# Lumina-Group/libzkp

Measured on NVIDIA B200. Metric: groth16_bn254_proofs_per_sec_batched, higher is better.
Workload: dtype u256 (8x32-bit Montgomery limbs, integer)

## Files before the change

libzkp_b200/csrc/ec.cuh:

```cuda
#pragma once
#include "field.cuh"

namespace lzkp {

template <class F>
struct Affine {
    F x, y;
    LZ_HD bool is_inf() const { return x.is_zero() && y.is_zero(); }
    LZ_HD static Affine inf() { return Affine{F::zero(), F::zero()}; }
    LZ_HD Affine neg() const { return Affine{x, y.neg()}; }
};

template <class F>
struct XYZZ {
    F x, y, zz, zzz;
    LZ_HD bool is_inf() const { return zz.is_zero(); }
    LZ_HD static XYZZ inf() { return XYZZ{F::one(), F::one(), F::zero(), F::zero()}; }
    LZ_HD static XYZZ from_affine(const Affine<F> &p) {
        if (p.is_inf()) return inf();
        return XYZZ{p.x, p.y, F::one(), F::one()};
    }
    LZ_HD XYZZ neg() const { return XYZZ{x, y.neg(), zz, zzz}; }

    LZ_COLD static XYZZ dbl_affine(const Affine<F> &p) {
        if (p.y.is_zero()) return inf();
        F U = p.y.dbl(), V = U.sqr(), W = U * V, S = p.x * V;
        F xx = p.x.sqr(), M = xx.dbl() + xx;
        XYZZ r;
        r.x = M.sqr() - S.dbl();
        r.y = F::msub(M, S - r.x, W, p.y);
        r.zz = V;
        r.zzz = W;
        return r;
    }
    LZ_HD void dbl() {
        if (is_inf()) return;
        if (y.is_zero()) { *this = inf(); return; }
        F U = y.dbl(), V = U.sqr(), W = U * V, S = x * V;
        F xx = x.sqr(), M = xx.dbl() + xx;
        F X3 = M.sqr() - S.dbl();
        F Y3 = F::msub(M, S - X3, W, y);
        x = X3; y = Y3;
        zz = V * zz;
        zzz = W * zzz;
    }
    LZ_COLD void dbl_cold() { dbl(); }
    LZ_COLD void add_cold(const XYZZ &q) { add(q); }
    LZ_COLD void madd_cold(const Affine<F> &p) { madd(p); }
    LZ_HD void madd(const Affine<F> &p) {
        if (p.is_inf()) return;
        if (is_inf()) { *this = from_affine(p); return; }
        F U2 = p.x * zz, S2 = p.y * zzz;
        F Pp = U2 - x, R = S2 - y;
        if (Pp.is_zero()) {
            if (R.is_zero()) *this = dbl_affine(p);
            else *this = inf();
            return;
        }
        F PP = Pp.sqr(), PPP = Pp * PP, Q = x * PP;
        F X3 = R.sqr() - PPP - Q.dbl();
        F Y3 = F::msub(R, Q - X3, y, PPP);
        x = X3; y = Y3;
        zz = zz * PP;
        zzz = zzz * PPP;
    }
    LZ_HD void madd_lazy(const Affine<F> &p) {
        if (p.is_inf()) return;
        if (zz.is_zero_2p()) { *this = from_affine(p); return; }
        F U2 = F::mul_lazy(p.x, zz), S2 = F::mul_lazy(p.y, zzz);
        F Pp = F::sub_2p(U2, x), R = F::sub_2p(S2, y);
        if (Pp.is_zero_2p()) {
            if (R.is_zero_2p()) *this = dbl_affine(p);
            else *this = inf();
            return;
        }
        F PP = Pp.sqr_lazy();
        F PPP = F::mul_lazy(Pp, PP), Q = F::mul_lazy(x, PP);
        F RR = R.sqr_lazy();
        F X3 = F::sub_2p(F::sub_2p(RR, PPP), F::add_2p(Q, Q));
        F Y3 = F::msub_lazy(R, F::sub_2p(Q, X3), y, PPP);
        x = X3; y = Y3;
        zz = F::mul_lazy(zz, PP);
        zzz = F::mul_lazy(zzz, PPP);
    }
    LZ_HD XYZZ canonical() const { return XYZZ{x.canonical(), y.canonical(), zz.canonical(), zzz.canonical()}; }
    LZ_HD void add(const XYZZ &q) {
        if (q.is_inf()) return;
        if (is_inf()) { *this = q; return; }
        F U1 = x * q.zz, U2 = q.x * zz, S1 = y * q.zzz, S2 = q.y * zzz;
        F Pp = U2 - U1, R = S2 - S1;
        if (Pp.is_zero()) {
            if (R.is_zero()) dbl_cold();
            else *this = inf();
            return;
        }
        F PP = Pp.sqr(), PPP = Pp * PP, Q = U1 * PP;
        F X3 = R.sqr() - PPP - Q.dbl();
        F Y3 = F::msub(R, Q - X3, S1, PPP);
        x = X3; y = Y3;
        zz = zz * q.zz * PP;
        zzz = zzz * q.zzz * PPP;
    }
    LZ_COLD Affine<F> to_affine() const {
        if (is_inf()) return Affine<F>::inf();
        F t = (zz * zzz).inverse();
        return Affine<F>{x * (t * zzz), y * (t * zz)};
    }
};

template <class F, int LIMBS>
LZ_COLD XYZZ<F> scalar_mul_window(const XYZZ<F> &p, const uint32_t (&k)[LIMBS]) {
    constexpr int NW = LIMBS * 8;
    static_assert(NW <= 64, "carry mask is 64 bits");
    XYZZ<F> T[8];
    T[0] = p;
    T[1] = p;
    T[1].dbl_cold();
#pragma unroll 1
    for (int i = 2; i < 8; i++) {
        T[i] = T[i - 1];
        T[i].add_cold(p);
    }
    uint64_t carries = 0;
    uint32_t c = 0;
#pragma unroll 1
    for (int i = 0; i < NW; i++) {
        const uint32_t v = ((k[i >> 3] >> ((i & 7) * 4)) & 15u) + c;
        c = v >= 8u ? 1u : 0u;
        carries |= (uint64_t)c << i;
    }
    XYZZ<F> acc = XYZZ<F>::inf();
#pragma unroll 1
    for (int i = NW; i >= 0; i--) {
        acc.dbl_cold(); acc.dbl_cold(); acc.dbl_cold(); acc.dbl_cold();
        int d;
        if (i == NW) d = (int)c;
        else {
            const uint32_t cin = i ? (uint32_t)(carries >> (i - 1)) & 1u : 0u, cout = (uint32_t)(carries >> i) & 1u;
            d = (int)(((k[i >> 3] >> ((i & 7) * 4)) & 15u) + cin) - (int)(16u * cout);
        }
        if (d != 0) {
            XYZZ<F> q = T[(d < 0 ? -d : d) - 1];
            if (d < 0) q.y = q.y.neg();
            acc.add_cold(q);
        }
    }
    return acc;
}
template <class F>
LZ_COLD XYZZ<F> scalar_mul(const XYZZ<F> &p, const Fr &k_canonical) {
    return scalar_mul_window<F, 8>(p, k_canonical.l);
}

struct GlvSplit {
    uint32_t k1[4], k2[4];
    bool neg1, neg2, ok;
};
template <int NO, int NA, int NB>
LZ_HD void mul_limbs(uint32_t (&out)[NO], const uint32_t (&a)[NA], const uint32_t (&b)[NB]) {
    uint64_t acc = 0, hi = 0;
#pragma unroll
    for (int k = 0; k < NO; k++) {
#pragma unroll
        for (int i = 0; i < NA; i++) {
            int j = k - i;
            if (j < 0 || j >= NB) continue;
            uint64_t p = (uint64_t)a[i] * b[j];
            acc += (uint32_t)p;
            hi += p >> 32;
        }
        out[k] = (uint32_t)acc;
        acc = (acc >> 32) + hi;
        hi = 0;
    }
}
LZ_HD GlvSplit glv_split(const Fr &k) {
    const uint32_t G1C[5] = {0x00ff6565u, 0x5398fd03u, 0xa773d2d2u, 0x4ccef014u, 0x00000002u};
    const uint32_t G2C[3] = {0xc7e0b3d7u, 0xd91d232eu, 0x00000002u};
    const uint32_t A1[4] = {0x7d4f1128u, 0x8211bbebu, 0xeeb859fcu, 0x6f4d8248u};
    const uint32_t A2[2] = {0x94d213e3u, 0x89d32568u};
    const uint32_t B2[4] = {0x1221250bu, 0x0be4e154u, 0xeeb859fdu, 0x6f4d8248u};
    uint32_t t13[13], t11[11], c1[5], c2[3];
    mul_limbs<13, 8, 5>(t13, k.l, G1C);
#pragma unroll
    for (int i = 0; i < 5; i++) c1[i] = t13[8 + i];
    mul_limbs<11, 8, 3>(t11, k.l, G2C);
#pragma unroll
    for (int i = 0; i < 3; i++) c2[i] = t11[8 + i];
    uint32_t p1[8], p2[8], p3[8], p4[8], k1[8], k2[8], t[8];
    mul_limbs<8, 5, 4>(p1, c1, A1);
    mul_limbs<8, 3, 2>(p2, c2, A2);
    mul_limbs<8, 5, 2>(p3, c1, A2);
    mul_limbs<8, 3, 4>(p4, c2, B2);
    sub8(t, k.l, p1);
    sub8(k1, t, p2);
    sub8(k2, p3, p4);
    GlvSplit o;
    o.neg1 = (k1[7] >> 31) != 0;
    o.neg2 = (k2[7] >> 31) != 0;
    uint32_t zero[8] = {0, 0, 0, 0, 0, 0, 0, 0};
    if (o.neg1) { sub8(t, zero, k1);
#pragma unroll
        for (int i = 0; i < 8; i++) k1[i] = t[i]; }
    if (o.neg2) { sub8(t, zero, k2);
#pragma unroll
        for (int i = 0; i < 8; i++) k2[i] = t[i]; }
    o.ok = (k1[4] | k1[5] | k1[6] | k1[7] | k2[4] | k2[5] | k2[6] | k2[7]) == 0;
#pragma unroll
    for (int i = 0; i < 4; i++) { o.k1[i] = k1[i]; o.k2[i] = k2[i]; }
    return o;
}
template <class F>
LZ_COLD XYZZ<F> scalar_mul_u128(const XYZZ<F> &p, const uint32_t (&k)[4]) {
    return scalar_mul_window<F, 4>(p, k);
}

static LZ_COLD XYZZ<Fq> scalar_mul_glv64(const XYZZ<Fq> &p, const uint32_t (&k)[4]) {
    XYZZ<Fq> T[8];
    T[0] = p;
    T[1] = p;
    T[1].dbl_cold();
#pragma unroll 1
    for (int i = 2; i < 8; i++) {
        T[i] = T[i - 1];
        T[i].add_cold(p);
    }
    Fq beta;
#pragma unroll
    for (int i = 0; i < 8; i++) beta.l[i] = FqParams::BETA(i);
    uint32_t carries[2] = {0, 0}, top[2] = {0, 0};
#pragma unroll 1
    for (int h = 0; h < 2; h++) {
        uint32_t c = 0;
#pragma unroll 1
        for (int i = 0; i < 16; i++) {
            const uint32_t v = ((k[2 * h + (i >> 3)] >> ((i & 7) * 4)) & 15u) + c;
            c = v >= 8u ? 1u : 0u;
            carries[h] |= c << i;
        }
        top[h] = c;
    }
    XYZZ<Fq> acc = XYZZ<Fq>::inf();
#pragma unroll 1
    for (int i = 16; i >= 0; i--) {
        acc.dbl_cold(); acc.dbl_cold(); acc.dbl_cold(); acc.dbl_cold();
#pragma unroll 1
        for (int h = 0; h < 2; h++) {
            int d;
            if (i == 16) d = (int)top[h];
            else {
                const uint32_t cin = i ? (carries[h] >> (i - 1)) & 1u : 0u, cout = (carries[h] >> i) & 1u;
                d = (int)(((k[2 * h + (i >> 3)] >> ((i & 7) * 4)) & 15u) + cin) - (int)(16u * cout);
            }
            if (d != 0) {
                XYZZ<Fq> q = T[(d < 0 ? -d : d) - 1];
                if (h) q.x = q.x * beta;
                if (d < 0) q.y = q.y.neg();
                acc.add_cold(q);
            }
        }
    }
    return acc;
}
LZ_HD Fr glv_lambda_mont() {
    const uint32_t v[8] = {0x55fcd653u, 0x0363f299u, 0x5fc1e200u, 0x73e7950bu, 0x576d9d24u, 0xc5fce83eu, 0xa1c3a4d4u, 0x059c805du};
    Fr r;
#pragma unroll
    for (int i = 0; i < 8; i++) r.l[i] = v[i];
    return r;
}
LZ_HD Fr glv64_coefficient(const uint32_t (&k)[4]) {
    Fr k1 = Fr::zero(), k2 = Fr::zero();
    k1.l[0] = k[0]; k1.l[1] = k[1];
    k2.l[0] = k[2]; k2.l[1] = k[3];
    return k1 + k2 * glv_lambda_mont();
}

using G1Affine = Affine<Fq>;
using G2Affine = Affine<Fq2>;
using G1XYZZ = XYZZ<Fq>;
using G2XYZZ = XYZZ<Fq2>;

static LZ_COLD bool g1_on_curve(const G1Affine &p) {
    if (p.is_inf()) return true;
    Fq b3;
#pragma unroll
    for (int i = 0; i < 8; i++) b3.l[i] = FqParams::B3(i);
    return p.y.sqr() == p.x.sqr() * p.x + b3;
}
static LZ_COLD bool g2_on_curve(const G2Affine &p) {
    if (p.is_inf()) return true;
    Fq2 b;
#pragma unroll
    for (int i = 0; i < 8; i++) { b.c0.l[i] = FqParams::G2B_C0(i); b.c1.l[i] = FqParams::G2B_C1(i); }
    return p.y.sqr() == p.x.sqr() * p.x + b;
}

}
```

libzkp_b200/csrc/field.cuh:

```cuda
#pragma once
#include <stdint.h>

#if defined(__CUDACC__)
#define LZ_HD __host__ __device__ __forceinline__
#define LZ_COLD __host__ __device__ __noinline__
#else
#define LZ_HD inline
#define LZ_COLD inline
#endif
#define LZ_CONST_ARRAY(NAME, ...)                                   \
    LZ_HD static constexpr uint32_t NAME(int i) {                   \
        const uint32_t v[8] = {__VA_ARGS__};                        \
        return v[i];                                                \
    }

#include "bn254_constants.cuh"

namespace lzkp {


LZ_HD void row_mul(uint32_t (&D)[8], uint32_t s0, uint32_t s1, uint32_t s2, uint32_t s3, uint32_t k) {
    const uint32_t s[4] = {s0, s1, s2, s3};
#pragma unroll
    for (int t = 0; t < 4; t++) {
// ... 340 lines not shown
        "addc.cc.u32 %7, %7, %17;\n\t"
        "addc.u32 %8, %18, %20;"
        : "+r"(mid[0]), "+r"(mid[1]), "+r"(mid[2]), "+r"(mid[3]), "+r"(mid[4]), "+r"(mid[5]), "+r"(mid[6]), "+r"(mid[7]),
          "=r"(mid[8]), "=&r"(junk)
        : "r"(x[0]), "r"(x[1]), "r"(x[2]), "r"(x[3]), "r"(x[4]), "r"(x[5]), "r"(x[6]), "r"(x[7]), "r"(c), "r"(n & 1u), "r"(n));
    asm("add.cc.u32 %0, %12, %24;\n\t"
        "addc.cc.u32 %1, %13, %25;\n\t"
        "addc.cc.u32 %2, %14, %26;\n\t"
        "addc.cc.u32 %3, %15, %27;\n\t"
        "addc.cc.u32 %4, %16, %28;\n\t"
        "addc.cc.u32 %5, %17, %29;\n\t"
        "addc.cc.u32 %6, %18, %30;\n\t"
        "addc.cc.u32 %7, %19, %31;\n\t"
        "addc.cc.u32 %8, %20, %32;\n\t"
        "addc.cc.u32 %9, %21, 0;\n\t"
        "addc.cc.u32 %10, %22, 0;\n\t"
        "addc.u32 %11, %23, 0;"
        : "=r"(T[4]), "=r"(T[5]), "=r"(T[6]), "=r"(T[7]), "=r"(T[8]), "=r"(T[9]), "=r"(T[10]), "=r"(T[11]), "=r"(T[12]),
          "=r"(T[13]), "=r"(T[14]), "=r"(T[15])
        : "r"(L[4]), "r"(L[5]), "r"(L[6]), "r"(L[7]), "r"(H[0]), "r"(H[1]), "r"(H[2]), "r"(H[3]), "r"(H[4]), "r"(H[5]),
          "r"(H[6]), "r"(H[7]),
          "r"(mid[0]), "r"(mid[1]), "r"(mid[2]), "r"(mid[3]), "r"(mid[4]), "r"(mid[5]), "r"(mid[6]), "r"(mid[7]), "r"(mid[8]));
#pragma unroll
    for (int i = 0; i < 4; i++) T[i] = L[i];
#else
    {
        uint64_t cy = n & 1u;
        for (int i = 0; i < 8; i++) {
            cy += (uint64_t)mid[i] + (M[i] ^ n);
            mid[i] = (uint32_t)cy;
            cy >>= 32;
        }
        mid[8] = (uint32_t)(c + n + cy);
        for (int i = 0; i < 4; i++) T[i] = L[i];
        cy = 0;
        for (int i = 4; i < 16; i++) {
            const uint32_t base = i < 8 ? L[i] : H[i - 8];
            cy += (uint64_t)base + (i - 4 < 9 ? mid[i - 4] : 0u);
            T[i] = (uint32_t)cy;
            cy >>= 32;
        }
    }
#endif
}

LZ_HD uint32_t red_shift_row(uint32_t &A0, uint32_t (&D)[8], uint32_t p1, uint32_t p3, uint32_t p5, uint32_t p7,
                             uint32_t inv) {
    uint32_t m;
#ifdef __CUDA_ARCH__
    asm("add.cc.u32 %0, %0, %2;\n\t"
        "mul.lo.u32 %9, %0, %14;\n\t"
        "madc.lo.cc.u32 %1, %10, %9, %3;\n\t"
        "madc.hi.cc.u32 %2, %10, %9, %4;\n\t"
        "madc.lo.cc.u32 %3, %11, %9, %5;\n\t"
        "madc.hi.cc.u32 %4, %11, %9, %6;\n\t"
        "madc.lo.cc.u32 %5, %12, %9, %7;\n\t"
        "madc.hi.cc.u32 %6, %12, %9, %8;\n\t"
        "madc.lo.cc.u32 %7, %13, %9, 0;\n\t"
        "madc.hi.u32 %8, %13, %9, 0;"
        : "+r"(A0), "+r"(D[0]), "+r"(D[1]), "+r"(D[2]), "+r"(D[3]), "+r"(D[4]), "+r"(D[5]), "+r"(D[6]), "+r"(D[7]), "=&r"(m)
        : "r"(p1), "r"(p3), "r"(p5), "r"(p7), "r"(inv));
#else
    const uint32_t s[4] = {p1, p3, p5, p7};
    uint64_t c = (uint64_t)A0 + D[1];
    A0 = (uint32_t)c;
    c >>= 32;
    m = A0 * inv;
    for (int t = 0; t < 4; t++) {
        uint64_t pr = (uint64_t)s[t] * m;
        uint32_t alo = t < 3 ? D[2 * t + 2] : 0, ahi = t < 3 ? D[2 * t + 3] : 0;
        uint64_t lo = (uint64_t)alo + (uint32_t)pr + c;
        uint64_t hi = (uint64_t)ahi + (uint32_t)(pr >> 32) + (lo >> 32);
        D[2 * t] = (uint32_t)lo;
        D[2 * t + 1] = (uint32_t)hi;
        c = hi >> 32;
    }
#endif
    return m;
}

template <class P>
LZ_HD void wide_fix_negative(uint32_t (&T)[16], uint32_t neg) {
    uint32_t hi[8], pm[8], fix[8];
#pragma unroll
    for (int i = 0; i < 8; i++) { hi[i] = T[8 + i]; pm[i] = neg ? P::MOD(i) : 0u; }
    add8(fix, hi, pm);
#pragma unroll
    for (int i = 0; i < 8; i++) T[8 + i] = fix[i];
}

template <class P>
struct alignas(16) Fp {
    uint32_t l[8];

    LZ_HD static Fp zero() {
        Fp r;
#pragma unroll
        for (int i = 0; i < 8; i++) r.l[i] = 0;
        return r;
    }
    LZ_HD static Fp one() {
        Fp r;
#pragma unroll
        for (int i = 0; i < 8; i++) r.l[i] = P::ONE(i);
        return r;
    }
    LZ_HD static Fp modulus() {
        Fp r;
#pragma unroll
        for (int i = 0; i < 8; i++) r.l[i] = P::MOD(i);
        return r;
    }
    LZ_HD static Fp r2() {
        Fp r;
#pragma unroll
        for (int i = 0; i < 8; i++) r.l[i] = P::R2(i);
        return r;
    }
    LZ_HD bool is_zero() const {
        uint32_t o = 0;
#pragma unroll
        for (int i = 0; i < 8; i++) o |= l[i];
        return o == 0;
    }
    LZ_HD bool operator==(const Fp &b) const {
        uint32_t o = 0;
#pragma unroll
        for (int i = 0; i < 8; i++) o |= l[i] ^ b.l[i];
        return o == 0;
    }
    LZ_HD bool operator!=(const Fp &b) const { return !(*this == b); }

    LZ_HD static Fp reduce_once(const uint32_t (&x)[8]) {
        Fp m = modulus(), d, r;
        uint32_t bw = sub8(d.l, x, m.l);
#pragma unroll
        for (int i = 0; i < 8; i++) r.l[i] = bw ? x[i] : d.l[i];
        return r;
    }
    LZ_HD friend Fp operator+(const Fp &a, const Fp &b) {
        uint32_t s[8];
        add8(s, a.l, b.l);
        return reduce_once(s);
    }
    LZ_HD friend Fp operator-(const Fp &a, const Fp &b) {
        Fp d, e, m = modulus(), r;
        uint32_t bw = sub8(d.l, a.l, b.l);
        add8(e.l, d.l, m.l);
#pragma unroll
        for (int i = 0; i < 8; i++) r.l[i] = bw ? e.l[i] : d.l[i];
        return r;
    }
    LZ_HD Fp neg() const {
        Fp m = modulus(), d, r;
        sub8(d.l, m.l, l);
        bool z = is_zero();
#pragma unroll
        for (int i = 0; i < 8; i++) r.l[i] = z ? 0u : d.l[i];
        return r;
    }
    LZ_HD Fp dbl() const { return *this + *this; }

    LZ_HD friend Fp operator*(const Fp &a, const Fp &b) { return reduce_once(mul_lazy(a, b).l); }
    LZ_HD Fp sqr() const { return reduce_once(sqr_lazy().l); }
    LZ_HD static Fp reduce_wide(const uint32_t (&T)[16]) { return reduce_once(reduce_wide_lazy(T).l); }
    LZ_HD static Fp msub(const Fp &a, const Fp &b, const Fp &c, const Fp &d) { return reduce_once(msub_lazy(a, b, c, d).l); }

    LZ_HD static Fp mul_lazy(const Fp &a, const Fp &b) {
        uint32_t X[8], Y[8];
        uint32_t m, c;
        row_mul(X, a.l[0], a.l[2], a.l[4], a.l[6], b.l[0]);
        row_mul(Y, a.l[1], a.l[3], a.l[5], a.l[7], b.l[0]);
        m = X[0] * P::INV;
        row_mad(Y, P::MOD(1), P::MOD(3), P::MOD(5), P::MOD(7), m);
        c = row_mad(X, P::MOD(0), P::MOD(2), P::MOD(4), P::MOD(6), m);
        Y[7] += c;
#pragma unroll
        for (int i = 1; i < 8; i++) {
            if (i & 1) {
                row_mad_shift(Y[0], X, a.l[1], a.l[3], a.l[5], a.l[7], b.l[i]);
                c = row_mad(Y, a.l[0], a.l[2], a.l[4], a.l[6], b.l[i]);
                X[7] += c;
                m = Y[0] * P::INV;
                row_mad(X, P::MOD(1), P::MOD(3), P::MOD(5), P::MOD(7), m);
                c = row_mad(Y, P::MOD(0), P::MOD(2), P::MOD(4), P::MOD(6), m);
                X[7] += c;
            } else {
                row_mad_shift(X[0], Y, a.l[1], a.l[3], a.l[5], a.l[7], b.l[i]);
                c = row_mad(X, a.l[0], a.l[2], a.l[4], a.l[6], b.l[i]);
                Y[7] += c;
                m = X[0] * P::INV;
                row_mad(Y, P::MOD(1), P::MOD(3), P::MOD(5), P::MOD(7), m);
                c = row_mad(X, P::MOD(0), P::MOD(2), P::MOD(4), P::MOD(6), m);
                Y[7] += c;
            }
        }
        uint32_t hi[8];
#pragma unroll
        for (int j = 0; j < 7; j++) hi[j] = Y[j + 1];
        hi[7] = 0;
        Fp s;
        add8(s.l, X, hi);
        return s;
    }
    LZ_HD Fp sqr_lazy() const {
#ifdef LZKP_SQR_AS_MUL
        return mul_lazy(*this, *this);
#endif
        uint32_t d[8], e[8];
        d[0] = l[0] << 1;
        e[0] = 0;
#pragma unroll
        for (int i = 1; i < 8; i++) { d[i] = (l[i] << 1) | (l[i - 1] >> 31); e[i] = l[i] << 1; }
        uint32_t t0 = 0, t1 = 0, t2 = 0, m[8];
        Fp r;
#pragma unroll
        for (int k = 0; k < 15; k++) {
#pragma unroll
            for (int i = 0; i < 8; i++) {
                const int j = k - i;
                if (j < i || j > 7) continue;
                if (j == i) mac3(t0, t1, t2, l[i], l[i]);
                else if (j == i + 1) mac3(t0, t1, t2, l[i], e[j]);
                else mac3(t0, t1, t2, l[i], d[j]);
            }
            if (k < 8) {
#pragma unroll
                for (int i = 0; i < k; i++) mac3(t0, t1, t2, m[i], P::MOD(k - i));
                m[k] = t0 * P::INV;
                mac3(t0, t1, t2, m[k], P::MOD(0));
            } else {
#pragma unroll
                for (int i = k - 7; i < 8; i++) mac3(t0, t1, t2, m[i], P::MOD(k - i));
                r.l[k - 8] = t0;
            }
            t0 = t1; t1 = t2; t2 = 0;
        }
        r.l[7] = t0;
        return r;
    }
    LZ_HD static Fp reduce_wide_lazy(const uint32_t (&T)[16]) {
        uint32_t X[8], Y[8];
        uint32_t m, c;
#pragma unroll
        for (int j = 0; j < 8; j++) X[j] = T[j];
        m = X[0] * P::INV;
        row_mul(Y, P::MOD(1), P::MOD(3), P::MOD(5), P::MOD(7), m);
        c = row_mad(X, P::MOD(0), P::MOD(2), P::MOD(4), P::MOD(6), m);
        Y[7] += c;
#pragma unroll
        for (int i = 1; i < 8; i++) {
            if (i & 1) {
                m = red_shift_row(Y[0], X, P::MOD(1), P::MOD(3), P::MOD(5), P::MOD(7), P::INV);
                c = row_mad(Y, P::MOD(0), P::MOD(2), P::MOD(4), P::MOD(6), m);
                X[7] += c;
            } else {
                m = red_shift_row(X[0], Y, P::MOD(1), P::MOD(3), P::MOD(5), P::MOD(7), P::INV);
                c = row_mad(X, P::MOD(0), P::MOD(2), P::MOD(4), P::MOD(6), m);
                Y[7] += c;
            }
        }
        uint32_t hi[8], th[8], u[8];
#pragma unroll
        for (int j = 0; j < 7; j++) hi[j] = Y[j + 1];
        hi[7] = 0;
#pragma unroll
        for (int j = 0; j < 8; j++) th[j] = T[8 + j];
        add8(u, X, hi);
        Fp s_;
        add8(s_.l, u, th);
        return s_;
    }
    LZ_HD static Fp msub_lazy(const Fp &a, const Fp &b, const Fp &c, const Fp &d) {
        uint32_t t0[16], t1[16];
        mul_wide(t0, a.l, b.l);
        mul_wide(t1, c.l, d.l);
        const uint32_t bw = sub16(t0, t0, t1);
        wide_fix_negative<P>(t0, bw);
        return reduce_wide_lazy(t0);
    }
    LZ_HD static Fp sub_2p(const Fp &a, const Fp &b) {
        Fp d, e, r;
        uint32_t bw = sub8(d.l, a.l, b.l);
        add8(e.l, d.l, modulus2().l);
#pragma unroll
        for (int i = 0; i < 8; i++) r.l[i] = bw ? e.l[i] : d.l[i];
        return r;
    }
    LZ_HD static Fp add_2p(const Fp &a, const Fp &b) {
        uint32_t s[8];
        Fp d, r;
        add8(s, a.l, b.l);
        uint32_t bw = sub8(d.l, s, modulus2().l);
#pragma unroll
        for (int i = 0; i < 8; i++) r.l[i] = bw ? s[i] : d.l[i];
        return r;
    }
    LZ_HD bool is_zero_2p() const {
        uint32_t z = 0, q = 0;
#pragma unroll
        for (int i = 0; i < 8; i++) { z |= l[i]; q |= l[i] ^ P::MOD(i); }
        return z == 0 || q == 0;
    }
    LZ_HD Fp canonical() const { return reduce_once(l); }
    LZ_HD static Fp modulus2() {
        Fp r;
#pragma unroll
        for (int i = 0; i < 8; i++) r.l[i] = (P::MOD(i) << 1) | (i ? P::MOD(i - 1) >> 31 : 0u);
        return r;
    }

    LZ_HD static Fp from_canonical(const Fp &c) { return c * r2(); }
    LZ_HD Fp to_canonical() const {
        Fp o = zero();
        o.l[0] = 1;
        return *this * o;
    }
    LZ_COLD Fp inverse() const {
        if (is_zero()) return zero();
        uint32_t u[8], v[8], x1[8], x2[8];
        const Fp m = modulus();
#pragma unroll
        for (int i = 0; i < 8; i++) { u[i] = l[i]; v[i] = m.l[i]; x1[i] = 0; x2[i] = 0; }
        x1[0] = 1;
        auto is_one = [](const uint32_t (&a)[8]) {
            uint32_t o = a[0] ^ 1u;
#pragma unroll
            for (int i = 1; i < 8; i++) o |= a[i];
            return o == 0;
        };
        auto shr1 = [](uint32_t (&a)[8]) {
#pragma unroll
            for (int i = 0; i < 7; i++) a[i] = (a[i] >> 1) | (a[i + 1] << 31);
            a[7] >>= 1;
        };
        auto halve_mod = [&](uint32_t (&x)[8]) {
            if (x[0] & 1u) { uint32_t t[8]; add8(t, x, m.l); 
#pragma unroll
                for (int i = 0; i < 8; i++) x[i] = t[i]; }
            shr1(x);
        };
        auto sub_mod = [&](uint32_t (&x)[8], const uint32_t (&y)[8]) {
            uint32_t d[8], e[8];
            uint32_t bw = sub8(d, x, y);
            add8(e, d, m.l);
#pragma unroll
            for (int i = 0; i < 8; i++) x[i] = bw ? e[i] : d[i];
        };
#pragma unroll 1
        while (!is_one(u) && !is_one(v)) {
#pragma unroll 1
            while (!(u[0] & 1u)) { shr1(u); halve_mod(x1); }
#pragma unroll 1
            while (!(v[0] & 1u)) { shr1(v); halve_mod(x2); }
            uint32_t d[8];
            if (sub8(d, u, v) == 0) {
#pragma unroll
                for (int i = 0; i < 8; i++) u[i] = d[i];
                sub_mod(x1, x2);
            } else {
                sub8(d, v, u);
#pragma unroll
                for (int i = 0; i < 8; i++) v[i] = d[i];
                sub_mod(x2, x1);
            }
        }
        Fp r, r3;
        const bool uu = is_one(u);
#pragma unroll
        for (int i = 0; i < 8; i++) { r.l[i] = uu ? x1[i] : x2[i]; r3.l[i] = P::R3(i); }
        return r * r3;
    }
    LZ_HD static bool gt_canonical(const Fp &a, const Fp &b) {
        uint32_t d[8];
        return sub8(d, b.l, a.l) != 0;
    }
};

using Fr = Fp<FrParams>;
using Fq = Fp<FqParams>;

struct Fq2;
#if !defined(LZKP_FQ2_INLINE) && defined(__CUDA_ARCH__)
static __device__ __noinline__ Fq2 fq2_mul_call(Fq2 a, Fq2 b);
static __device__ __noinline__ Fq2 fq2_sqr_call(Fq2 a);
#endif
struct Fq2 {
    Fq c0, c1;
    LZ_HD static Fq2 zero() { return Fq2{Fq::zero(), Fq::zero()}; }
    LZ_HD static Fq2 one() { return Fq2{Fq::one(), Fq::zero()}; }
    LZ_HD bool is_zero() const { return c0.is_zero() && c1.is_zero(); }
    LZ_HD bool operator==(const Fq2 &b) const { return c0 == b.c0 && c1 == b.c1; }
    LZ_HD bool operator!=(const Fq2 &b) const { return !(*this == b); }
    LZ_HD friend Fq2 operator+(const Fq2 &a, const Fq2 &b) { return Fq2{a.c0 + b.c0, a.c1 + b.c1}; }
    LZ_HD friend Fq2 operator-(const Fq2 &a, const Fq2 &b) { return Fq2{a.c0 - b.c0, a.c1 - b.c1}; }
    LZ_HD Fq2 neg() const { return Fq2{c0.neg(), c1.neg()}; }
    LZ_HD Fq2 dbl() const { return Fq2{c0.dbl(), c1.dbl()}; }
    LZ_HD friend Fq2 operator*(const Fq2 &a, const Fq2 &b) {
#if !defined(LZKP_FQ2_INLINE) && defined(__CUDA_ARCH__)
        return fq2_mul_call(a, b);
#elif defined(LZKP_FQ2_SCHOOLBOOK)
        return Fq2{a.c0 * b.c0 - a.c1 * b.c1, a.c0 * b.c1 + a.c1 * b.c0};
#else
        Fq v0 = a.c0 * b.c0, v1 = a.c1 * b.c1;
        Fq s = (a.c0 + a.c1) * (b.c0 + b.c1);
        return Fq2{v0 - v1, s - v0 - v1};
#endif
    }
    LZ_HD Fq2 sqr() const {
#if !defined(LZKP_FQ2_INLINE) && defined(__CUDA_ARCH__)
        return fq2_sqr_call(*this);
#endif
        Fq m = c0 * c1;
        return Fq2{(c0 + c1) * (c0 - c1), m.dbl()};
    }
    LZ_HD static Fq2 msub(const Fq2 &a, const Fq2 &b, const Fq2 &c, const Fq2 &d) { return a * b - c * d; }
    LZ_HD Fq2 inverse() const {
        Fq n = (c0.sqr() + c1.sqr()).inverse();
        return Fq2{c0 * n, (c1 * n).neg()};
    }
};
LZ_HD Fq2 fq2_mul_lazy(const Fq2 &a, const Fq2 &b) {
    uint32_t t0[16], t1[16], t2[16], sa[8], sb[8];
    mul_wide(t0, a.c0.l, b.c0.l);
    mul_wide(t1, a.c1.l, b.c1.l);
    add8(sa, a.c0.l, a.c1.l);
    add8(sb, b.c0.l, b.c1.l);
    mul_wide(t2, sa, sb);
    sub16(t2, t2, t0);
    sub16(t2, t2, t1);
    const uint32_t bw = sub16(t0, t0, t1);
    uint32_t hi[8], pm[8], fix[8];
#pragma unroll
    for (int i = 0; i < 8; i++) { hi[i] = t0[8 + i]; pm[i] = bw ? FqParams::MOD(i) : 0u; }
    add8(fix, hi, pm);
#pragma unroll
    for (int i = 0; i < 8; i++) t0[8 + i] = fix[i];
    return Fq2{Fq::reduce_wide(t0), Fq::reduce_wide(t2)};
}
#if !defined(LZKP_FQ2_INLINE) && defined(__CUDA_ARCH__)
static __device__ __noinline__ Fq2 fq2_mul_call(Fq2 a, Fq2 b) { return fq2_mul_lazy(a, b); }
static __device__ __noinline__ Fq2 fq2_sqr_call(Fq2 a) {
    Fq m = a.c0 * a.c1;
    return Fq2{(a.c0 + a.c1) * (a.c0 - a.c1), m.dbl()};
}
#endif

}
```

libzkp_b200/csrc/msm_batch.cu:

```cuda
#include <algorithm>
#include <cstdlib>
#include "tables.h"
#include "dev_util.cuh"

#ifndef LZKP_G2_MINB
#define LZKP_G2_MINB 6
#endif
#ifndef LZKP_G1_MINB
#define LZKP_G1_MINB 4
#endif
#define LZKP_G2_MINB_SEL(F) (sizeof(F) == sizeof(::lzkp::Fq) ? LZKP_G1_MINB : LZKP_G2_MINB)
namespace lzkp {

template <class F, int BLOCK, class DigT>
__global__ void __launch_bounds__(BLOCK, LZKP_G2_MINB_SEL(F)) k_msm_batch(const Affine<F> *__restrict__ table, uint32_t N,
                                                     const uint32_t *__restrict__ unit_dig,
                                                     const uint32_t *__restrict__ unit_tbl,
                                                     const uint2 *__restrict__ items, const DigT *__restrict__ dig,
                                                     uint32_t P, XYZZ<F> *__restrict__ partial) {
    const uint32_t p = blockIdx.x * BLOCK + threadIdx.x, item = blockIdx.y;
    if (p >= P) return;
    const uint2 range = items[item];
    constexpr bool lazy = sizeof(F) == sizeof(Fq);
    XYZZ<F> acc = XYZZ<F>::inf();
    int d = dig[(size_t)__ldg(unit_dig + range.x) * P + p];
    Affine<F> pt = Affine<F>::inf();
    if (d) pt = gather_point(table, N, __ldg(unit_tbl + range.x), d);
    for (uint32_t u = range.x; u < range.y; u++) {
        int dn = 0;
        Affine<F> ptn = Affine<F>::inf();
        if (u + 1 < range.y) {
            dn = dig[(size_t)__ldg(unit_dig + u + 1) * P + p];
            if (dn) ptn = gather_point(table, N, __ldg(unit_tbl + u + 1), dn);
        }
        if (d) {
            if constexpr (lazy) acc.madd_lazy(pt);
            else acc.madd(pt);
        }
        d = dn;
        pt = ptn;
    }
    if constexpr (lazy) acc = acc.canonical();
    st_vec(partial + (size_t)item * P + p, acc);
}
template <class F>
__global__ void __launch_bounds__(128) k_msm_reduce1(XYZZ<F> *partial, const uint2 *msm_items, uint32_t P, uint32_t G) {
    uint32_t p = blockIdx.x * blockDim.x + threadIdx.x, q = blockIdx.y, g = blockIdx.z;
    if (p >= P) return;
    uint2 r = msm_items[q];
    if (r.x + g >= r.y) return;
    XYZZ<F> acc = ld_vec(partial + (size_t)(r.x + g) * P + p);
    for (uint32_t it = r.x + g + G; it < r.y; it += G) acc.add_cold(ld_vec(partial + (size_t)it * P + p));
    st_vec(partial + (size_t)(r.x + g) * P + p, acc);
}
template <class F>
__global__ void __launch_bounds__(128) k_msm_reduce(const XYZZ<F> *partial, const uint2 *msm_items, uint32_t P,
                                                    uint32_t G, XYZZ<F> *out) {
    uint32_t p = blockIdx.x * blockDim.x + threadIdx.x, q = blockIdx.y;
    if (p >= P) return;
    uint2 r = msm_items[q];
    uint32_t end = min(r.y, r.x + G);
    XYZZ<F> acc = XYZZ<F>::inf();
    for (uint32_t it = r.x; it < end; it++) acc.add_cold(ld_vec(partial + (size_t)it * P + p));
    st_vec(out + (size_t)q * P + p, acc);
}

template <class F>
__global__ void __launch_bounds__(128) k_msm_fold(XYZZ<F> *partial, const uint2 *msm_items, uint32_t P, uint32_t half,
                                                  XYZZ<F> *out) {
    uint32_t p = blockIdx.x * blockDim.x + threadIdx.x, q = blockIdx.y, g = blockIdx.z;
    if (p >= P) return;
    const uint2 r = msm_items[q];
    const uint32_t live = min(r.y - r.x, 2 * half);
    if (g >= live) {
        if (half == 1 && g == 0) st_vec(out + (size_t)q * P + p, XYZZ<F>::inf());
        return;
    }
    XYZZ<F> acc = ld_vec(partial + (size_t)(r.x + g) * P + p);
    if (g + half < live) acc.add_cold(ld_vec(partial + (size_t)(r.x + g + half) * P + p));
    if (half == 1) st_vec(out + (size_t)q * P + p, acc);
    else st_vec(partial + (size_t)(r.x + g) * P + p, acc);
}

template <class F, int T>
__global__ void __launch_bounds__(T) k_msm_reduce_tree(const XYZZ<F> *__restrict__ partial, const uint2 *__restrict__ msm_items,
                                                       uint32_t P, XYZZ<F> *__restrict__ out) {
    __shared__ uint4 raw[T * sizeof(XYZZ<F>) / 16];
    XYZZ<F> *sm = reinterpret_cast<XYZZ<F> *>(raw);
    const uint32_t p = blockIdx.x, q = blockIdx.y, t = threadIdx.x;
    const uint2 r = msm_items[q];
    XYZZ<F> acc = XYZZ<F>::inf();
    for (uint32_t it = r.x + t; it < r.y; it += T) acc.add_cold(ld_vec(partial + (size_t)it * P + p));
    st_vec(sm + t, acc);
    __syncthreads();
    for (uint32_t s = T / 2; s > 0; s >>= 1) {
        if (t < s) {
            XYZZ<F> a = ld_vec(sm + t);
            a.add_cold(ld_vec(sm + t + s));
            st_vec(sm + t, a);
        }
        __syncthreads();
    }
    if (t == 0) st_vec(out + (size_t)q * P + p, ld_vec(sm));
}

}

namespace lzkp {
namespace eng {
uint32_t small_batch_limit() {
    static const uint32_t v = [] {
        const char *e = getenv("LZKP_SMALL_BATCH");
        return e ? (uint32_t)atoi(e) : 512u;
    }();
    return v;
}

int batch_msm_g1_resident(uint32_t dig_bytes, uint32_t *out) {
    int dev = 0, sms = 0, per_sm = 0;
    CUDA_TRY(cudaGetDevice(&dev));
    CUDA_TRY(cudaDeviceGetAttribute(&sms, cudaDevAttrMultiProcessorCount, dev));
    if (dig_bytes == 2) CUDA_TRY(cudaOccupancyMaxActiveBlocksPerMultiprocessor(&per_sm, k_msm_batch<Fq, 128, int16_t>, 128, 0));
    else CUDA_TRY(cudaOccupancyMaxActiveBlocksPerMultiprocessor(&per_sm, k_msm_batch<Fq, 128, int32_t>, 128, 0));
    *out = (uint32_t)std::max(1, sms * per_sm);
    return LZKP_OK;
}

void batch_msm_g1_items(const BatchMsmArgs &a, uint32_t item0, uint32_t count, cudaStream_t st) {
    if (!count) return;
    if (a.P <= small_batch_limit()) {
        if (a.dig_bytes == 2)
            LAUNCH((k_msm_batch<Fq, 32, int16_t>), dim3((a.P + 31) / 32, count), 32, 0, st, (const G1Affine *)a.table, a.N, a.unit_dig, a.unit_tbl,
                   (const uint2 *)a.items + item0, (const int16_t *)a.dig, a.P, (G1XYZZ *)a.partial + (size_t)item0 * a.P);
        else
            LAUNCH((k_msm_batch<Fq, 32, int32_t>), dim3((a.P + 31) / 32, count), 32, 0, st, (const G1Affine *)a.table, a.N, a.unit_dig, a.unit_tbl,
                   (const uint2 *)a.items + item0, (const int32_t *)a.dig, a.P, (G1XYZZ *)a.partial + (size_t)item0 * a.P);
        return;
    }
    if (a.dig_bytes == 2)
        LAUNCH((k_msm_batch<Fq, 128, int16_t>), dim3((a.P + 127) / 128, count), 128, 0, st, (const G1Affine *)a.table, a.N, a.unit_dig,
               a.unit_tbl, (const uint2 *)a.items + item0, (const int16_t *)a.dig, a.P, (G1XYZZ *)a.partial + (size_t)item0 * a.P);
    else
        LAUNCH((k_msm_batch<Fq, 128, int32_t>), dim3((a.P + 127) / 128, count), 128, 0, st, (const G1Affine *)a.table, a.N, a.unit_dig,
               a.unit_tbl, (const uint2 *)a.items + item0, (const int32_t *)a.dig, a.P, (G1XYZZ *)a.partial + (size_t)item0 * a.P);
}
constexpr uint32_t kReduceFan = 8;
void batch_msm_g1_reduce(const BatchMsmArgs &a, cudaStream_t st) {
    if (a.P <= small_batch_limit()) {
        LAUNCH((k_msm_reduce_tree<Fq, 128>), dim3(a.P, a.n_msm), 128, 0, st, (const G1XYZZ *)a.partial, (const uint2 *)a.msm_items,
               a.P, (G1XYZZ *)a.out);
        return;
    }
    LAUNCH((k_msm_reduce1<Fq>), dim3((a.P + 127) / 128, a.n_msm, kReduceFan), 128, 0, st, (G1XYZZ *)a.partial,
           (const uint2 *)a.msm_items, a.P, kReduceFan);
    for (uint32_t half = kReduceFan / 2; half >= 1; half >>= 1)
        LAUNCH((k_msm_fold<Fq>), dim3((a.P + 127) / 128, a.n_msm, half), 128, 0, st, (G1XYZZ *)a.partial,
               (const uint2 *)a.msm_items, a.P, half, (G1XYZZ *)a.out);
}
void batch_msm_g1(const BatchMsmArgs &a, cudaStream_t st) {
    batch_msm_g1_items(a, 0, a.n_items, st);
    batch_msm_g1_reduce(a, st);
}
void batch_msm_g2(const BatchMsmArgs &a, cudaStream_t st) {
    if (a.P <= small_batch_limit()) {
        if (a.dig_bytes == 2)
            LAUNCH((k_msm_batch<Fq2, 32, int16_t>), dim3((a.P + 31) / 32, a.n_items), 32, 0, st, (const G2Affine *)a.table, a.N, a.unit_dig,
                   a.unit_tbl, (const uint2 *)a.items, (const int16_t *)a.dig, a.P, (G2XYZZ *)a.partial);
        else
            LAUNCH((k_msm_batch<Fq2, 32, int32_t>), dim3((a.P + 31) / 32, a.n_items), 32, 0, st, (const G2Affine *)a.table, a.N, a.unit_dig,
                   a.unit_tbl, (const uint2 *)a.items, (const int32_t *)a.dig, a.P, (G2XYZZ *)a.partial);
        LAUNCH((k_msm_reduce_tree<Fq2, 128>), dim3(a.P, a.n_msm), 128, 0, st, (const G2XYZZ *)a.partial, (const uint2 *)a.msm_items,
               a.P, (G2XYZZ *)a.out);
        return;
    }
    if (a.dig_bytes == 2)
        LAUNCH((k_msm_batch<Fq2, 64, int16_t>), dim3((a.P + 63) / 64, a.n_items), 64, 0, st, (const G2Affine *)a.table, a.N,
               a.unit_dig, a.unit_tbl, (const uint2 *)a.items, (const int16_t *)a.dig, a.P, (G2XYZZ *)a.partial);
    else
        LAUNCH((k_msm_batch<Fq2, 64, int32_t>), dim3((a.P + 63) / 64, a.n_items), 64, 0, st, (const G2Affine *)a.table, a.N,
               a.unit_dig, a.unit_tbl, (const uint2 *)a.items, (const int32_t *)a.dig, a.P, (G2XYZZ *)a.partial);
    LAUNCH((k_msm_reduce1<Fq2>), dim3((a.P + 127) / 128, a.n_msm, 2 * kReduceFan), 128, 0, st, (G2XYZZ *)a.partial,
           (const uint2 *)a.msm_items, a.P, 2 * kReduceFan);
    for (uint32_t half = kReduceFan; half >= 1; half >>= 1)
        LAUNCH((k_msm_fold<Fq2>), dim3((a.P + 127) / 128, a.n_msm, half), 128, 0, st, (G2XYZZ *)a.partial,
               (const uint2 *)a.msm_items, a.P, half, (G2XYZZ *)a.out);
}

}
}
```

Measured before the change: 183,900.

## Add G2 MSM kernel with cp.async staged point prefetch and lazy Fq2 arithmetic

Adds a dedicated G2 batched-MSM kernel that prefetches the table points for upcoming digits into a shared-memory double buffer using cp.async, and applies the digit sign inside a new signed lazy mixed addition. Fq2 gains lazy (2p-range) mul/sqr/add/sub helpers, so G2 accumulation skips the full reductions, and the reduce kernels canonicalise G2 partials when loading them. This is meant to hide global gather latency and cut modular-reduction work in the G2 hot loop. In exchange it uses more shared memory per block, which may lower occupancy. The negation path and lazy-range invariants also add correctness risk.

```diff
diff --git a/libzkp_b200/csrc/ec.cuh b/libzkp_b200/csrc/ec.cuh
--- a/libzkp_b200/csrc/ec.cuh
+++ b/libzkp_b200/csrc/ec.cuh
@@ -82,6 +82,34 @@
         x = X3; y = Y3;
         zz = F::mul_lazy(zz, PP);
         zzz = F::mul_lazy(zzz, PPP);
+    }
+    template <class Pt>
+    LZ_HD void madd_lazy_signed(const Pt &p, bool neg) {
+        if (zz.is_zero_2p()) { *this = from_affine(signed_point(p, neg)); return; }
+        F U2 = F::mul_lazy(p.x(), zz);
+        F Pp = F::sub_2p(U2, x);
+        F y2 = p.y();
+        if (neg) y2 = y2.neg_2p();
+        F R = F::sub_2p(F::mul_lazy(y2, zzz), y);
+        if (Pp.is_zero_2p()) {
+            if (R.is_zero_2p()) *this = dbl_affine(signed_point(p, neg));
+            else *this = inf();
+            return;
+        }
+        F PP = Pp.sqr_lazy();
+        zz = F::mul_lazy(zz, PP);
+        F PPP = F::mul_lazy(Pp, PP);
+        zzz = F::mul_lazy(zzz, PPP);
+        F Q = F::mul_lazy(x, PP);
+        F X3 = F::sub_2p(F::sub_2p(R.sqr_lazy(), PPP), F::add_2p(Q, Q));
+        F Y3 = F::sub_2p(F::mul_lazy(R, F::sub_2p(Q, X3)), F::mul_lazy(y, PPP));
+        x = X3; y = Y3;
+    }
+    template <class Pt>
+    LZ_HD static Affine<F> signed_point(const Pt &p, bool neg) {
+        Affine<F> a = p.point();
+        if (neg) a.y = a.y.neg();
+        return a;
     }
     LZ_HD XYZZ canonical() const { return XYZZ{x.canonical(), y.canonical(), zz.canonical(), zzz.canonical()}; }
     LZ_HD void add(const XYZZ &q) {
diff --git a/libzkp_b200/csrc/field.cuh b/libzkp_b200/csrc/field.cuh
--- a/libzkp_b200/csrc/field.cuh
+++ b/libzkp_b200/csrc/field.cuh
@@ -666,6 +666,11 @@
         for (int i = 0; i < 8; i++) { z |= l[i]; q |= l[i] ^ P::MOD(i); }
         return z == 0 || q == 0;
     }
+    LZ_HD Fp neg_2p() const {
+        Fp r;
+        sub8(r.l, modulus().l, l);
+        return r;
+    }
     LZ_HD Fp canonical() const { return reduce_once(l); }
     LZ_HD static Fp modulus2() {
         Fp r;
@@ -748,7 +753,11 @@
 #if !defined(LZKP_FQ2_INLINE) && defined(__CUDA_ARCH__)
 static __device__ __noinline__ Fq2 fq2_mul_call(Fq2 a, Fq2 b);
 static __device__ __noinline__ Fq2 fq2_sqr_call(Fq2 a);
-#endif
+static __device__ __noinline__ Fq2 fq2_mul_lazy_call(Fq2 a, Fq2 b);
+static __device__ __noinline__ Fq2 fq2_sqr_lazy_call(Fq2 a);
+#endif
+LZ_HD Fq2 fq2_mul_2p(const Fq2 &a, const Fq2 &b);
+LZ_HD Fq2 fq2_sqr_2p(const Fq2 &a);
 struct Fq2 {
     Fq c0, c1;
     LZ_HD static Fq2 zero() { return Fq2{Fq::zero(), Fq::zero()}; }
@@ -783,24 +792,51 @@
         Fq n = (c0.sqr() + c1.sqr()).inverse();
         return Fq2{c0 * n, (c1 * n).neg()};
     }
+
+    LZ_HD static Fq2 mul_lazy(const Fq2 &a, const Fq2 &b) {
+#if !defined(LZKP_FQ2_INLINE) && defined(__CUDA_ARCH__)
+        return fq2_mul_lazy_call(a, b);
+#else
+        return fq2_mul_2p(a, b);
+#endif
+    }
+    LZ_HD Fq2 sqr_lazy() const {
+#if !defined(LZKP_FQ2_INLINE) && defined(__CUDA_ARCH__)
+        return fq2_sqr_lazy_call(*this);
+#else
+        return fq2_sqr_2p(*this);
+#endif
+    }
+    LZ_HD static Fq2 sub_2p(const Fq2 &a, const Fq2 &b) { return Fq2{Fq::sub_2p(a.c0, b.c0), Fq::sub_2p(a.c1, b.c1)}; }
+    LZ_HD static Fq2 add_2p(const Fq2 &a, const Fq2 &b) { return Fq2{Fq::add_2p(a.c0, b.c0), Fq::add_2p(a.c1, b.c1)}; }
+    LZ_HD bool is_zero_2p() const { return c0.is_zero_2p() && c1.is_zero_2p(); }
+    LZ_HD Fq2 neg_2p() const { return Fq2{c0.neg_2p(), c1.neg_2p()}; }
+    LZ_HD Fq2 canonical() const { return Fq2{c0.canonical(), c1.canonical()}; }
 };
-LZ_HD Fq2 fq2_mul_lazy(const Fq2 &a, const Fq2 &b) {
-    uint32_t t0[16], t1[16], t2[16], sa[8], sb[8];
-    mul_wide(t0, a.c0.l, b.c0.l);
-    mul_wide(t1, a.c1.l, b.c1.l);
+LZ_HD Fq2 fq2_mul_wide_lazy(const Fq2 &a, const Fq2 &b) {
+    uint32_t t[16], u[16], s[16], sa[8], sb[8];
+    mul_wide(t, a.c0.l, b.c0.l);
+    mul_wide(u, a.c1.l, b.c1.l);
+    add16(s, t, u);
+    wide_fix_negative<FqParams>(t, sub16(t, t, u));
+    const Fq c0 = Fq::reduce_wide_lazy(t);
     add8(sa, a.c0.l, a.c1.l);
     add8(sb, b.c0.l, b.c1.l);
-    mul_wide(t2, sa, sb);
-    sub16(t2, t2, t0);
-    sub16(t2, t2, t1);
-    const uint32_t bw = sub16(t0, t0, t1);
-    uint32_t hi[8], pm[8], fix[8];
-#pragma unroll
-    for (int i = 0; i < 8; i++) { hi[i] = t0[8 + i]; pm[i] = bw ? FqParams::MOD(i) : 0u; }
-    add8(fix, hi, pm);
-#pragma unroll
-    for (int i = 0; i < 8; i++) t0[8 + i] = fix[i];
-    return Fq2{Fq::reduce_wide(t0), Fq::reduce_wide(t2)};
+    mul_wide(u, sa, sb);
+    sub16(u, u, s);
+    return Fq2{c0, Fq::reduce_wide_lazy(u)};
+}
+LZ_HD Fq2 fq2_mul_lazy(const Fq2 &a, const Fq2 &b) {
+    const Fq2 r = fq2_mul_wide_lazy(a, b);
+    return Fq2{r.c0.canonical(), r.c1.canonical()};
+}
+LZ_HD Fq2 fq2_mul_2p(const Fq2 &a, const Fq2 &b) {
+    const Fq2 r = fq2_mul_wide_lazy(a, b);
+    return Fq2{r.c0, Fq::reduce_once(r.c1.l)};
+}
+LZ_HD Fq2 fq2_sqr_2p(const Fq2 &a) {
+    const Fq m = Fq::mul_lazy(a.c0, a.c1);
+    return Fq2{Fq::mul_lazy(Fq::add_2p(a.c0, a.c1), Fq::sub_2p(a.c0, a.c1)), Fq::add_2p(m, m)};
 }
 #if !defined(LZKP_FQ2_INLINE) && defined(__CUDA_ARCH__)
 static __device__ __noinline__ Fq2 fq2_mul_call(Fq2 a, Fq2 b) { return fq2_mul_lazy(a, b); }
@@ -808,6 +844,8 @@
     Fq m = a.c0 * a.c1;
     return Fq2{(a.c0 + a.c1) * (a.c0 - a.c1), m.dbl()};
 }
-#endif
-
-}
+static __device__ __noinline__ Fq2 fq2_mul_lazy_call(Fq2 a, Fq2 b) { return fq2_mul_2p(a, b); }
+static __device__ __noinline__ Fq2 fq2_sqr_lazy_call(Fq2 a) { return fq2_sqr_2p(a); }
+#endif
+
+}
diff --git a/libzkp_b200/csrc/msm_batch.cu b/libzkp_b200/csrc/msm_batch.cu
--- a/libzkp_b200/csrc/msm_batch.cu
+++ b/libzkp_b200/csrc/msm_batch.cu
@@ -3,17 +3,16 @@
 #include "tables.h"
 #include "dev_util.cuh"
 
+#ifndef LZKP_G1_MINB
+#define LZKP_G1_MINB 4
+#endif
 #ifndef LZKP_G2_MINB
 #define LZKP_G2_MINB 6
 #endif
-#ifndef LZKP_G1_MINB
-#define LZKP_G1_MINB 4
-#endif
-#define LZKP_G2_MINB_SEL(F) (sizeof(F) == sizeof(::lzkp::Fq) ? LZKP_G1_MINB : LZKP_G2_MINB)
 namespace lzkp {
 
 template <class F, int BLOCK, class DigT>
-__global__ void __launch_bounds__(BLOCK, LZKP_G2_MINB_SEL(F)) k_msm_batch(const Affine<F> *__restrict__ table, uint32_t N,
+__global__ void __launch_bounds__(BLOCK, LZKP_G1_MINB) k_msm_batch(const Affine<F> *__restrict__ table, uint32_t N,
                                                      const uint32_t *__restrict__ unit_dig,
                                                      const uint32_t *__restrict__ unit_tbl,
                                                      const uint2 *__restrict__ items, const DigT *__restrict__ dig,
@@ -21,7 +20,6 @@
     const uint32_t p = blockIdx.x * BLOCK + threadIdx.x, item = blockIdx.y;
     if (p >= P) return;
     const uint2 range = items[item];
-    constexpr bool lazy = sizeof(F) == sizeof(Fq);
     XYZZ<F> acc = XYZZ<F>::inf();
     int d = dig[(size_t)__ldg(unit_dig + range.x) * P + p];
     Affine<F> pt = Affine<F>::inf();
@@ -33,15 +31,77 @@
             dn = dig[(size_t)__ldg(unit_dig + u + 1) * P + p];
             if (dn) ptn = gather_point(table, N, __ldg(unit_tbl + u + 1), dn);
         }
+        if (d) acc.madd_lazy(pt);
+        d = dn;
+        pt = ptn;
+    }
+    acc = acc.canonical();
+    st_vec(partial + (size_t)item * P + p, acc);
+}
+
+__device__ __forceinline__ void cp_async16(void *smem, const void *gmem) {
+    asm volatile("cp.async.cg.shared.global [%0], [%1], 16;" ::"r"((uint32_t)__cvta_generic_to_shared(smem)), "l"(gmem)
+                 : "memory");
+}
+__device__ __forceinline__ void cp_async_commit() { asm volatile("cp.async.commit_group;" ::: "memory"); }
+template <int N>
+__device__ __forceinline__ void cp_async_wait() { asm volatile("cp.async.wait_group %0;" ::"n"(N) : "memory"); }
+
+template <int BLOCK>
+struct StagedG2 {
+    const uint4 *s;
+    __device__ __forceinline__ Fq2 ld(int c) const {
+        Fq2 r;
+        uint4 *d = reinterpret_cast<uint4 *>(&r);
+#pragma unroll
+        for (int i = 0; i < 4; i++) d[i] = s[(c + i) * BLOCK];
+        return r;
+    }
+    __device__ __forceinline__ Fq2 x() const { return ld(0); }
+    __device__ __forceinline__ Fq2 y() const { return ld(4); }
+    __device__ __forceinline__ G2Affine point() const { return G2Affine{x(), y()}; }
+};
+
+template <int BLOCK, class DigT>
+__global__ void __launch_bounds__(BLOCK, LZKP_G2_MINB) k_msm_batch_g2(const G2Affine *__restrict__ table, uint32_t N,
+                                                                   const uint32_t *__restrict__ unit_dig,
+                                                                   const uint32_t *__restrict__ unit_tbl,
+                                                                   const uint2 *__restrict__ items, const DigT *__restrict__ dig,
+                                                                   uint32_t P, G2XYZZ *__restrict__ partial) {
+    __shared__ uint4 ring[2][8][BLOCK];
+    const uint32_t t = threadIdx.x, p = blockIdx.x * BLOCK + t, item = blockIdx.y;
+    if (p >= P) return;
+    const uint2 range = items[item];
+    auto stage = [&](int slot, uint32_t u, int d) {
+        const uint4 *src = reinterpret_cast<const uint4 *>(table + (size_t)__ldg(unit_tbl + u) * N + (uint32_t)(abs(d) - 1));
+#pragma unroll
+        for (int c = 0; c < 8; c++) cp_async16(&ring[slot][c][t], src + c);
+    };
+    auto digit = [&](uint32_t u) { return u < range.y ? (int)dig[(size_t)__ldg(unit_dig + u) * P + p] : 0; };
+    G2XYZZ acc = G2XYZZ::inf();
+    int d = digit(range.x), dn = digit(range.x + 1);
+    if (d) stage(0, range.x, d);
+    cp_async_commit();
+    int slot = 0;
+    for (uint32_t u = range.x; u < range.y; u++) {
+        const int dnn = digit(u + 2);
+        if (dn) stage(slot ^ 1, u + 1, dn);
+        cp_async_commit();
         if (d) {
-            if constexpr (lazy) acc.madd_lazy(pt);
-            else acc.madd(pt);
+            cp_async_wait<1>();
+            acc.madd_lazy_signed(StagedG2<BLOCK>{&ring[slot][0][t]}, d < 0);
         }
         d = dn;
-        pt = ptn;
-    }
-    if constexpr (lazy) acc = acc.canonical();
+        dn = dnn;
+        slot ^= 1;
+    }
     st_vec(partial + (size_t)item * P + p, acc);
+}
+
+template <class F>
+__device__ __forceinline__ XYZZ<F> ld_partial(const XYZZ<F> *p) {
+    if constexpr (sizeof(F) == sizeof(Fq2)) return ld_vec(p).canonical();
+    else return ld_vec(p);
 }
 template <class F>
 __global__ void __launch_bounds__(128) k_msm_reduce1(XYZZ<F> *partial, const uint2 *msm_items, uint32_t P, uint32_t G) {
@@ -49,8 +109,8 @@
     if (p >= P) return;
     uint2 r = msm_items[q];
     if (r.x + g >= r.y) return;
-    XYZZ<F> acc = ld_vec(partial + (size_t)(r.x + g) * P + p);
-    for (uint32_t it = r.x + g + G; it < r.y; it += G) acc.add_cold(ld_vec(partial + (size_t)it * P + p));
+    XYZZ<F> acc = ld_partial(partial + (size_t)(r.x + g) * P + p);
+    for (uint32_t it = r.x + g + G; it < r.y; it += G) acc.add_cold(ld_partial(partial + (size_t)it * P + p));
     st_vec(partial + (size_t)(r.x + g) * P + p, acc);
 }
 template <class F>
@@ -90,7 +150,7 @@
     const uint32_t p = blockIdx.x, q = blockIdx.y, t = threadIdx.x;
     const uint2 r = msm_items[q];
     XYZZ<F> acc = XYZZ<F>::inf();
-    for (uint32_t it = r.x + t; it < r.y; it += T) acc.add_cold(ld_vec(partial + (size_t)it * P + p));
+    for (uint32_t it = r.x + t; it < r.y; it += T) acc.add_cold(ld_partial(partial + (size_t)it * P + p));
     st_vec(sm + t, acc);
     __syncthreads();
     for (uint32_t s = T / 2; s > 0; s >>= 1) {
@@ -164,20 +224,20 @@
 void batch_msm_g2(const BatchMsmArgs &a, cudaStream_t st) {
     if (a.P <= small_batch_limit()) {
         if (a.dig_bytes == 2)
-            LAUNCH((k_msm_batch<Fq2, 32, int16_t>), dim3((a.P + 31) / 32, a.n_items), 32, 0, st, (const G2Affine *)a.table, a.N, a.unit_dig,
+            LAUNCH((k_msm_batch_g2<32, int16_t>), dim3((a.P + 31) / 32, a.n_items), 32, 0, st, (const G2Affine *)a.table, a.N, a.unit_dig,
                    a.unit_tbl, (const uint2 *)a.items, (const int16_t *)a.dig, a.P, (G2XYZZ *)a.partial);
         else
-            LAUNCH((k_msm_batch<Fq2, 32, int32_t>), dim3((a.P + 31) / 32, a.n_items), 32, 0, st, (const G2Affine *)a.table, a.N, a.unit_dig,
+            LAUNCH((k_msm_batch_g2<32, int32_t>), dim3((a.P + 31) / 32, a.n_items), 32, 0, st, (const G2Affine *)a.table, a.N, a.unit_dig,
                    a.unit_tbl, (const uint2 *)a.items, (const int32_t *)a.dig, a.P, (G2XYZZ *)a.partial);
         LAUNCH((k_msm_reduce_tree<Fq2, 128>), dim3(a.P, a.n_msm), 128, 0, st, (const G2XYZZ *)a.partial, (const uint2 *)a.msm_items,
                a.P, (G2XYZZ *)a.out);
         return;
     }
     if (a.dig_bytes == 2)
-        LAUNCH((k_msm_batch<Fq2, 64, int16_t>), dim3((a.P + 63) / 64, a.n_items), 64, 0, st, (const G2Affine *)a.table, a.N,
+        LAUNCH((k_msm_batch_g2<64, int16_t>), dim3((a.P + 63) / 64, a.n_items), 64, 0, st, (const G2Affine *)a.table, a.N,
                a.unit_dig, a.unit_tbl, (const uint2 *)a.items, (const int16_t *)a.dig, a.P, (G2XYZZ *)a.partial);
     else
-        LAUNCH((k_msm_batch<Fq2, 64, int32_t>), dim3((a.P + 63) / 64, a.n_items), 64, 0, st, (const G2Affine *)a.table, a.N,
+        LAUNCH((k_msm_batch_g2<64, int32_t>), dim3((a.P + 63) / 64, a.n_items), 64, 0, st, (const G2Affine *)a.table, a.N,
                a.unit_dig, a.unit_tbl, (const uint2 *)a.items, (const int32_t *)a.dig, a.P, (G2XYZZ *)a.partial);
     LAUNCH((k_msm_reduce1<Fq2>), dim3((a.P + 127) / 128, a.n_msm, 2 * kReduceFan), 128, 0, st, (G2XYZZ *)a.partial,
            (const uint2 *)a.msm_items, a.P, 2 * kReduceFan);
```

Measured after the change: 185,600, median of 6. No clear change (+0.9%).
